# prequel-dev/plz4

Measured on AMD Instinct MI355X. Metric: MiB/s enc+dec, 4MiB independent blocks, level 1, block-checksum on (duplex steps over 2 streams), higher is better.
Workload: dtype u8

## Files before the change

plz4_amd/_native.py:

```python
from __future__ import annotations

import ctypes as C
import os

import numpy as np

HERE = os.path.dirname(os.path.abspath(__file__))
LIB_PATH = os.path.join(HERE, "libplz4hip.so")

ABI_VERSION = 2
SYMBOLS = [
    "plz4hip_abi_version", "plz4hip_device_count", "plz4hip_ctx_create", "plz4hip_ctx_destroy",
    "plz4hip_last_error", "plz4hip_compress_bound", "plz4hip_compress_batch", "plz4hip_decompress_batch",
    "plz4hip_xxh32_batch", "plz4hip_encode_records", "plz4hip_decode_records", "plz4hip_dev_stage_stride",
    "plz4hip_dev_encode_records", "plz4hip_dev_compact_records", "plz4hip_dev_scatter_records",
    "plz4hip_dev_decode_records", "plz4hip_dev_decode_records_ex", "plz4hip_dev_duplex_records", "plz4hip_dev_encode_body", "plz4hip_dev_duplex_body", "plz4hip_dev_encode_records_ex", "plz4hip_dev_encode_body_ex", "plz4hip_dev_compress", "plz4hip_dev_decompress", "plz4hip_ctx_trim",
    "plz4hip_ctx_counters",
    "plz4hip_dev_resident_waves", "plz4hip_dict_create", "plz4hip_dict_destroy", "plz4hip_compress_batch_dict", "plz4hip_decode_records_chains",
    "plz4hip_decompress_batch_dict", "plz4hip_encode_records_ex", "plz4hip_decode_records_ex",
    "plz4hip_xxh32_stream_create", "plz4hip_xxh32_stream_destroy", "plz4hip_xxh32_stream_reset", "plz4hip_xxh32_stream_update",
    "plz4hip_dev_xxh32_stream_update", "plz4hip_xxh32_stream_sum", "plz4hip_ctx_set_content_hash",
    "plz4hip_mgpu_create", "plz4hip_mgpu_destroy", "plz4hip_mgpu_count", "plz4hip_mgpu_ctx", "plz4hip_mgpu_last_error",
    "plz4hip_mgpu_compress_batch", "plz4hip_mgpu_decompress_batch", "plz4hip_mgpu_encode_records", "plz4hip_mgpu_decode_records",
    "plz4hip_mgpu_dev_encode_frame", "plz4hip_mgpu_dev_decode_frame",
# ... 363 lines not shown
    def hash_reset(self, h):
        self._chk(self.L.plz4hip_xxh32_stream_reset(self.h, h))

    def hash_update(self, h, buf: np.ndarray):
        buf = np.ascontiguousarray(buf)
        self._chk(self.L.plz4hip_xxh32_stream_update(self.h, h, buf.ctypes.data if buf.size else None, buf.size))

    def dev_hash_update(self, h, ptr, n, stream=0):
        self._chk(self.L.plz4hip_dev_xxh32_stream_update(self.h, h, ptr, n, stream))

    def hash_sum(self, h) -> int:
        out = C.c_uint32()
        self._chk(self.L.plz4hip_xxh32_stream_sum(self.h, h, C.byref(out)))
        return int(out.value)

    def set_content_hash(self, h):
        self._chk(self.L.plz4hip_ctx_set_content_hash(self.h, h))

    def trim(self):
        self._chk(self.L.plz4hip_ctx_trim(self.h))

    COUNTERS = ("fx_blocks", "fx_rounds_last", "fx_pieces_again", "dx_blocks", "dxl_blocks", "dxl_rounds_last", "dxl_groups_last",
                "fxl_blocks", "l1x_blocks", "hcx_blocks", "dx_big_blocks", "dx_big_rounds_last", "dx_big_runs_last",
                "mx_blocks", "mx_rounds_last", "mx_pieces_again", "mxl_blocks")

    def counters(self) -> dict:
        out = (C.c_int64 * len(self.COUNTERS))()
        rc = int(self.L.plz4hip_ctx_counters(self.h, out, len(self.COUNTERS)))
        if rc < 0:
            self._chk(rc)
        return {k: int(out[i]) for i, k in enumerate(self.COUNTERS)}


class MultiEngine:

    def __init__(self, devices):
        self.L = load()
        arr = (C.c_int * len(devices))(*devices)
        h = C.c_void_p()
        rc = self.L.plz4hip_mgpu_create(arr, len(devices), C.byref(h))
        if rc != 0:
            raise EngineError(rc, "plz4hip_mgpu_create")
        self.h = h
        self.g = len(devices)

    def close(self):
        if getattr(self, "h", None):
# ... 58 lines not shown
```

plz4_amd/csrc/plz4hip.hip:

```cpp
#include <hip/hip_runtime.h>

#include <array>
#include <atomic>
#include <mutex>
#include <thread>
#include <string>
#include <vector>
#include <cstdio>
#include <cstring>

#include "../../include/plz4hip.h"
#include "stream_ws.h"
#if defined(PLZ4_STATS)
__device__ unsigned long long plz4_stats[24];
#endif
#include "lz4_device.inl"
#include "lz4_seq_device.inl"
#include "lz4hc_device.inl"
#include "lz4hc12_device.inl"
#include "lz4hc_lazy_device.inl"
#include "lz4hcx_device.inl"
#include "lz4_dx_device.inl"
#include "lz4_fx_device.inl"
#include "lz4_mx_device.inl"
// ... 93 lines not shown
    ENC_WAVE_TABLE(lds);
    for (int i = next_block(a.queue); i < a.nBlocks; i = next_block(a.queue)) {
        const int      n   = block_len(a, i);
        const uint8_t* s   = a.src + (int64_t)i * a.srcStride;
        uint8_t*       rec = a.dst + (int64_t)i * a.dstStride;
        int      c    = wave_encode_block(s, n, rec + 4, a.bsz, lds);
        uint32_t word = (uint32_t)c & 0x7FFFFFFFu;
        if (c == 0) {
            wave_copy(rec + 4, s, n);
            c = n;
            word = 0x80000000u | ((uint32_t)n & 0x7FFFFFFFu);
        }
        int len = c + 4;
        if (a.blockChecksum) {
            WAVE_FENCE();
            const uint32_t x = wave_xxh32(rec + 4, c);
            if ((threadIdx.x & 63u) == 0) st32u(rec + 4 + c, x);
            len += 4;
        }
        if ((threadIdx.x & 63u) == 0) { st32u(rec, word); a.result[i] = len; }
    }
}

template <int kLdsWin = 0>
__device__ __forceinline__ void l1_parse_loop(const CodecArgs& a, uint32_t* lds, uint8_t* scr = nullptr)
{
    for (int i = next_block(a.queue); i < a.nBlocks; i = next_block(a.queue)) {
        const int gi = a.blk0 + i;
        const int n  = block_len(a, gi);
        int lastAnchor = 0, nseq = -1;
        if (n >= 0 && n <= a.l1MaxLen)
            nseq = wave_parse_l1<kLdsWin>(a.src + (int64_t)gi * a.srcStride, n, lds, a.l1Seq + (int64_t)i * a.l1SeqStride, &lastAnchor, scr);
        if ((threadIdx.x & 63u) == 0) { SeqInfo inf; inf.nseq = nseq; inf.lastAnchor = lastAnchor; inf.total = 0; inf.stored = 0; a.l1Info[i] = inf; }
    }
    if (a.gate && (threadIdx.x & 63u) == 0) atomicMax(a.gate, a.gateSeq);
}
__global__ __launch_bounds__(64) void k_parse_gate(const uint32_t* gate, uint32_t want)
{
    for (int it = 0; it < 400000; ++it) {
        if ((int32_t)(__hip_atomic_load(gate, __ATOMIC_RELAXED, __HIP_MEMORY_SCOPE_AGENT) - want) >= 0) break;
        __builtin_amdgcn_s_sleep(127);
    }
}
template <int W> __global__ __launch_bounds__(64 * W) void k_l1_parse(CodecArgs a)
{
    ENC_WAVE_TABLE(lds);
    l1_parse_loop<2>(a, lds);
}

template <bool kBack, bool kSeg = false> __device__ __forceinline__ void l1_sizes_body(const CodecArgs a, const FxlBlk* xb = nullptr)
{
    const int i = blockIdx.y, wave = blockIdx.x * 4 + (int)(threadIdx.x >> 6), nW = gridDim.x * 4;
    const int nseq = a.l1Info[i].nseq;
    if (nseq <= 0) return;
    const int gi = a.blk0 + i;
    const uint8_t*  s   = a.src + (int64_t)gi * a.srcStride;
    const uint64_t* seq = a.l1Seq + (int64_t)i * a.l1SeqStride;
    const int nChunks = (nseq + kSeqChunk - 1) / kSeqChunk;
    for (int c = wave; c < nChunks; c += nW) {
        const uint32_t v = seq_emit_sizes<kBack, kSeg>(s, seq, kBack ? a.l1Bk + (int64_t)i * a.l1SeqStride : nullptr, nseq, c, kSeg ? max_(xb[i].pfx, 0) : 0);
        if ((threadIdx.x & 63u) == 0) a.l1ChunkBytes[(int64_t)i * a.l1MaxChunks + c] = v;
    }
}
template <bool kBack> __global__ __launch_bounds__(256) void k_l1_sizes(CodecArgs a) { l1_sizes_body<kBack>(a); }

__global__ __launch_bounds__(256) void k_l1_scan(CodecArgs a)
{
    const int i = blockIdx.x * 4 + (int)(threadIdx.x >> 6);
    if (i >= a.nBlocks) return;
    const int gi = a.blk0 + i;
    const int n  = block_len(a, gi);
    SeqInfo inf = a.l1Info[i];
    const int cap = a.rawMode ? (a.dstCap ? a.dstCap[gi] : a.dstCapAll) : a.bsz;
    int total = 0;
    const bool broken = inf.nseq == kSeqEngineFailed;
    if (inf.nseq >= 0)
        total = seq_emit_scan(a.l1ChunkBytes + (int64_t)i * a.l1MaxChunks, a.l1ChunkOff + (int64_t)i * a.l1MaxChunks, inf.nseq, inf.lastAnchor, n, cap);
    if ((threadIdx.x & 63u) == 0) {
        inf.total = total; inf.stored = (total == 0);
        a.l1Info[i] = inf;
        if (broken) a.result[gi] = PLZ4HIP_E_DEVICE;
        else if (a.rawMode) a.result[gi] = total;
        else if (a.bodyOff) {
            a.result[gi] = (total ? total : n) + 4 + (a.blockChecksum ? 4 : 0);
        } else {
            const int c = total ? total : n;
            st32u(a.dst + (int64_t)gi * a.dstStride, total ? ((uint32_t)c & 0x7FFFFFFFu) : (0x80000000u | ((uint32_t)n & 0x7FFFFFFFu)));
// ... 1257 lines not shown
    wave_xxh32_x16(p, n, x);
    if ((threadIdx.x & 3u) == 0 && i < a.nBlocks) {
        const int st = n[0] < 0 ? PLZ4HIP_BLK_SIZE_OVERFLOW : x[0] != want ? PLZ4HIP_BLK_HASH_MISMATCH : PLZ4HIP_BLK_OK;
        a.status[i] = st;
        if (st != PLZ4HIP_BLK_OK) a.result[i] = 0;
    }
}
#if defined(PLZ4_EXP_DEC_EU)
__global__ __launch_bounds__(64) __attribute__((amdgpu_waves_per_eu(5, 6))) void k_decode_rec(CodecArgs a)
#else
__global__ __launch_bounds__(64) __attribute__((amdgpu_waves_per_eu(6, 6))) void k_decode_rec(CodecArgs a)
#endif
{
    __shared__ __attribute__((aligned(16))) uint8_t dl[kDecLdsBytes];
    decode_rec_loop<false>(a, dl);
}
__global__ __launch_bounds__(64) void k_decode_rec_dx(CodecArgs a)
{
    __shared__ __attribute__((aligned(16))) uint8_t dl[kDecLdsBytes];
    decode_rec_loop<true>(a, dl);
}

constexpr int kWinScratch = 256;
constexpr int duplex_wgs_per_cu(int P, int D) { return (160 * 1024) / (P * (kHashBytes + kWinScratch) + D * kDecLdsBytes); }
#if defined(PLZ4_EXP_DUPLEX_EU)
constexpr int duplex_waves_per_eu(int P, int D) { return PLZ4_EXP_DUPLEX_EU; }
#else
constexpr int duplex_waves_per_eu(int P, int D) { return ((P + D) * duplex_wgs_per_cu(P, D) + 3) / 4; }
#endif
template <int P, int D, int PRIO> __global__ __launch_bounds__(64 * (P + D))
__attribute__((amdgpu_waves_per_eu(duplex_waves_per_eu(P, D), duplex_waves_per_eu(P, D))))
void k_l1_duplex(CodecArgs a, CodecArgs d)
{
    __shared__ uint32_t tabS[P][kHashBytes / 4];
    __shared__ __attribute__((aligned(16))) uint8_t dlS[D][kDecLdsBytes];
    __shared__ __attribute__((aligned(16))) uint8_t winS[P][kWinScratch];
    const int w = plz4_readfirstlane((int)(threadIdx.x >> 6));
    if (w < P) {
        if (PRIO) __builtin_amdgcn_s_setprio(PRIO);
        l1_parse_loop<1>(a, tabS[w], winS[w]);
    } else {
        decode_rec_loop<false>(d, dlS[w - P]);
    }
}

__global__ __launch_bounds__(64) void k_xxh32(const uint8_t* base, int64_t stride, const int32_t* len, uint32_t* out,
                                              int n, uint32_t* queue)
{
    for (int i = next_block(queue); i < n; i = next_block(queue)) {
        const uint32_t x = wave_xxh32(base + (int64_t)i * stride, len[i]);
        if ((threadIdx.x & 63u) == 0) out[i] = x;
    }
}

__global__ __launch_bounds__(64) void k_xxh32_stream(XxhStream* st, const uint8_t* base, int64_t stride, const int32_t* lens, int n, int64_t single, int reset)
{
    if (reset) wave_xxh32_stream_reset(st);
    if (!lens) { wave_xxh32_stream_update(st, base, single); return; }
    for (int i = 0; i < n; ++i) {
        const int len = plz4_readfirstlane(lens[i]);
        if (len > 0) wave_xxh32_stream_update(st, base + (int64_t)i * stride, len);
    }
}

__global__ __launch_bounds__(64) void k_scan(const int32_t* __restrict__ len, int64_t* __restrict__ off, int n)
// ... 51 lines not shown
    int          cus = 0;
    int          encWaves = 0, decWaves = 0;
    struct HostSlot { uint8_t* h = nullptr; size_t hcap = 0; uint8_t* d = nullptr; size_t dcap = 0; hipStream_t s = nullptr;
                      hipEvent_t evData = nullptr, evHash = nullptr; bool hashBusy = false; DeviceBuffer l1; };
    plz4hip_xxh32_stream* contentHash = nullptr;
    static constexpr int kSlots = 3;
    HostSlot     slot[kSlots];
    DeviceBuffer hc;  int hcWaves = 0;
    DeviceBuffer h12;  int h12ParseWaves = 0;  int h12SegWaves = 0;  int hcLazyWaves = 0;  size_t h12ErrOff = 0;
    StreamOrder  hcOrder;
    hipStream_t  hashStream = nullptr;
    static constexpr int kL1Shared = 2;
    DeviceBuffer l1[kL1Shared];  StreamOrder l1Order[kL1Shared];
    int          l1Refused = 0;
    uint32_t*    d_gate = nullptr; uint32_t gateSeq = 0; hipStream_t gateStream = nullptr; bool gatePending = false; int gateBlocks = 0;
    hipStream_t  hcBuildStream = nullptr; hipEvent_t evHcFork = nullptr, evHcHist = nullptr, evHcChain[2] = {nullptr, nullptr}, evHcFree[2] = {nullptr, nullptr};
    DeviceBuffer hcPfx;  int hcLazyExWaves = 0;
    int hcxWaves[4] = {0, 0, 0, 0};
    DeviceBuffer dx;  StreamOrder dxOrder;
    hipStream_t  dxHashStream = nullptr; hipEvent_t evDxFork = nullptr, evDxHash = nullptr;
    DeviceBuffer fx;  StreamOrder fxOrder;
    DeviceBuffer mx;  StreamOrder mxOrder;
    DeviceBuffer xstage;  StreamOrder xstageOrder;
    static constexpr int kCounters = 17;
    unsigned long long* d_counters = nullptr;
    DeviceBuffer lenCopy;  StreamOrder lenOrder;
    DeviceBuffer chainCopy;  StreamOrder chainOrder;
    struct Owned { DeviceBuffer* buf; StreamOrder* order; bool trimmed; };
    std::array<Owned, 11> owned()
    {
        return {{{&hc, &hcOrder, true}, {&h12, &hcOrder, true}, {&hcPfx, &hcOrder, false}, {&l1[0], &l1Order[0], true},
                 {&l1[1], &l1Order[1], true}, {&dx, &dxOrder, true}, {&fx, &fxOrder, true}, {&lenCopy, &lenOrder, false},
                 {&chainCopy, &chainOrder, false}, {&xstage, &xstageOrder, true}, {&mx, &mxOrder, true}}};
    }
};

struct plz4hip_xxh32_stream { XxhStream* d_state = nullptr; hipEvent_t done = nullptr; };

struct plz4hip_dict {
    uint8_t*  d_bytes = nullptr;  int len = 0;
    uint32_t* d_table = nullptr;
    uint8_t*  d_hc = nullptr;
    uint8_t*  d_hcx = nullptr;
    std::vector<uint8_t> h_bytes;
};

namespace {

// ... 165 lines not shown
    a.l1Seq = (uint64_t*)a.h12F; a.l1SeqStride = L.fStride; a.l1MaxChunks = L.maxChunks; a.l1Bk = nullptr;
    a.l1Info = (SeqInfo*)(base + L.offInfo) + k;
    a.l1ChunkBytes = (uint32_t*)(base + L.offChunkB) + k * L.maxChunks; a.l1ChunkOff = (uint32_t*)(base + L.offChunkO) + k * L.maxChunks;
    a.lzRecStride = L.recStride;
    a.lzRec = (uint64_t*)(base + L.offRec) + k * L.recStride; a.lzBridge = (uint64_t*)(base + L.offBridge) + k * L.recStride;
    a.lzMeta = (LzSegMeta*)(base + L.offMeta) + k * kLzMaxSegs; a.lzStarts = (uint64_t*)(base + L.offStarts) + k * kLzMaxSegs * kLzStarts;
    a.lzPieces = (LzPiece*)(base + L.offPieces) + k * 2 * kLzMaxSegs;
}

void bind_hc_pre(CodecArgs& a, uint8_t* base, const HcPreLayout& L, bool lists)
{
    a.h12Chain = (uint16_t*)(base + L.offChain); a.h12ChainStride = L.stride;
    a.h12Rank = lists ? (uint32_t*)(base + L.offRank) : nullptr;
    a.h12List = lists ? (uint32_t*)(base + L.offList) : nullptr;
    a.h12Offsets = lists ? (uint32_t*)(base + L.offOffsets) : nullptr;
}

L1Switches read_l1_switches() { return parse_l1_switches([](const char* n) { return (const char*)getenv(n); }); }
MxSwitches read_mx_switches() { return parse_mx_switches([](const char* n) { return (const char*)getenv(n); }); }
HcSwitches read_hc_switches() { return parse_hc_switches([](const char* n) { return (const char*)getenv(n); }); }
DxSwitches read_dx_switches() { return parse_dx_switches([](const char* n) { return (const char*)getenv(n); }); }

enum class Emit { Back, Mid, Seg };
void launch_emit(hipStream_t s, const CodecArgs& a, int ng, int g0, int maxChunks, Emit kind, const FxlBlk* xb = nullptr, bool ctxSmall = false)
{
    int wg = (16384 / ng) / 4;
    if (wg > (maxChunks + 3) / 4) wg = (maxChunks + 3) / 4;
    if (wg < 1) wg = 1;
    if (kind == Emit::Seg) hipLaunchKernelGGL(k_fxl_sizes, dim3(wg, ng), dim3(256), 0, s, a, xb);
    else if (kind == Emit::Mid) hipLaunchKernelGGL(k_l1_sizes<false>, dim3(wg, ng), dim3(256), 0, s, a);
    else hipLaunchKernelGGL(k_l1_sizes<true>, dim3(wg, ng), dim3(256), 0, s, a);
    hipLaunchKernelGGL(k_l1_scan, dim3((ng + 3) / 4), dim3(256), 0, s, a);
    if (ctxSmall && a.bodyOff) hipLaunchKernelGGL(k_fxl_small, dim3(ng < 1024 ? ng : 1024), dim3(64), 0, s, a);
    if (a.bodyOff) hipLaunchKernelGGL(k_scan_from, dim3(1), dim3(64), 0, s, (const int32_t*)(a.result + g0), a.bodyOff + g0, ng, g0 == 0 ? 1 : 0);
    if (kind == Emit::Seg) hipLaunchKernelGGL(k_fxl_write, dim3(wg, ng), dim3(256), 0, s, a, xb);
    else if (kind == Emit::Mid) hipLaunchKernelGGL(k_l1_write<false>, dim3(wg, ng), dim3(256), 0, s, a);
    else hipLaunchKernelGGL(k_l1_write<true>, dim3(wg, ng), dim3(256), 0, s, a);
    if (!a.rawMode && a.blockChecksum) hipLaunchKernelGGL(k_l1_finish, dim3((ng + 15) / 16), dim3(64), 0, s, a);
    if (ctxSmall && !a.bodyOff) hipLaunchKernelGGL(k_fxl_small, dim3(ng < 1024 ? ng : 1024), dim3(64), 0, s, a);
}

void launch_rec_verify(hipStream_t s, const CodecArgs& d)
{
    if (d.blockChecksum && d.nBlocks > 0) hipLaunchKernelGGL(k_rec_verify16, dim3((d.nBlocks + 15) / 16), dim3(64), 0, s, d);
}
int launch_l1(plz4hip_ctx* c, hipStream_t s, CodecArgs a, int nb, int maxLen, int rawMode, DeviceBuffer* ws, bool* midDeclined = nullptr,
              const CodecArgs* rider = nullptr, bool hist = false, bool l1x = false, const L1Switches* read = nullptr);

int launch_hc_body(plz4hip_ctx* c, hipStream_t s, const HcSwitches& sw, CodecArgs a, int nb, int maxLen, int rawMode, bool* forked);
int launch_hc(plz4hip_ctx* c, hipStream_t s, CodecArgs a, int nb, int maxLen, int rawMode)
{
    const HcSwitches sw = read_hc_switches();
    HIPCHK(c, c->hcOrder.wait(s));
    MarkOnExit job;
// ... 249 lines not shown
{
    const int nws = sw.oneWorkspace ? 1 : plz4hip_ctx::kL1Shared;
    int mine = -1, idle = -1, fresh = -1;
    for (int i = 0; i < nws; ++i) {
        if (c->l1[i].d && c->l1Order[i].stream == s && mine < 0) mine = i;
        if (c->l1[i].d && idle < 0 && c->l1Order[i].idle()) idle = i;
        if (!c->l1[i].d && fresh < 0) fresh = i;
    }
    return mine >= 0 ? mine : (idle >= 0 ? idle : (fresh >= 0 ? fresh : 0));
}

int l1_gate(plz4hip_ctx* c, hipStream_t s, CodecArgs& a, int ng)
{
    if (c->gatePending && c->gateStream != s && c->gateBlocks >= 8 * c->cus)
        hipLaunchKernelGGL(k_parse_gate, dim3(1), dim3(64), 0, s, (const uint32_t*)c->d_gate, c->gateSeq);
    if (c->gateSeq >= 0x7FFF0000u) {
        HIPCHK(c, hipDeviceSynchronize()); HIPCHK(c, zero_sync(c, c->d_gate, sizeof(uint32_t))); c->gateSeq = 0;
    }
    a.gate = c->d_gate; a.gateSeq = ++c->gateSeq;
    c->gatePending = true; c->gateStream = s; c->gateBlocks = ng;
    return PLZ4HIP_OK;
}

int launch_duplex(plz4hip_ctx* c, hipStream_t s, const L1Switches& sw, const CodecArgs& a, const CodecArgs& rider, int ng)
{
    const int P = sw.duplexP, D = sw.duplexD;
#define DUPLEX_CASE(PP, DD) \
    if (P == PP && D == DD) { \
        int wgs = ((ng + PP - 1) / PP > (rider.nBlocks + DD - 1) / DD) ? (ng + PP - 1) / PP : (rider.nBlocks + DD - 1) / DD; \
        const int hold = c->cus * duplex_wgs_per_cu(PP, DD); \
        if (wgs > hold) wgs = hold; \
        if (sw.duplexPrio) hipLaunchKernelGGL((k_l1_duplex<PP, DD, 3>), dim3(wgs), dim3(64 * (PP + DD)), 0, s, a, rider); \
        else               hipLaunchKernelGGL((k_l1_duplex<PP, DD, 0>), dim3(wgs), dim3(64 * (PP + DD)), 0, s, a, rider); \
        return PLZ4HIP_OK; \
    }
    DUPLEX_CASE(1, 1) DUPLEX_CASE(1, 2) DUPLEX_CASE(3, 4) DUPLEX_CASE(9, 7)
#undef DUPLEX_CASE
    return fail(c, PLZ4HIP_E_ARG, "PLZ4HIP_DUPLEX: not a built combination");
}

int launch_l1(plz4hip_ctx* c, hipStream_t s, CodecArgs a, int nb, int maxLen, int rawMode, DeviceBuffer* ws, bool* midDeclined,
              const CodecArgs* rider, bool hist, bool l1x, const L1Switches* read)
{
    hipError_t e;
    const L1Switches sw = read ? *read : read_l1_switches();
    const bool mid = midDeclined != nullptr;
    const L1Shape shape{nb, maxLen, rawMode != 0, mid, rider != nullptr, hist, l1x, a.bodyOff != nullptr, hist && a.dictLen >= 8};
    const L1Want want = l1_want(shape, sw);
    const bool mxl = mid && a.hcPfx != nullptr;
    const MxShape mxShape{a.level, nb, maxLen, a.hcEx != 0 || a.hcPfx != nullptr, rider != nullptr};
    const MxWant mxWant = !mid ? MxWant{} : mxl ? mxl_want(mxShape, read_mx_switches()) : mx_want(mxShape, read_mx_switches());
    a.rawMode = rawMode; a.blk0 = 0; a.nBlocks = nb;
    const bool shared = (ws == nullptr);
    int wsi = 0;
    if (shared) { wsi = pick_l1_workspace(c, s, sw); ws = &c->l1[wsi]; }
    bool granted = want.staged;
    const auto need_for = [&](int per) { return l1_layout(per, maxLen, l1x).total; };
    int per = nb;
    if (shared && granted && wsi != 0 && !ws->d && c->l1Refused > 0) { c->l1Refused--; wsi = 0; ws = &c->l1[0]; }
    if (shared && granted && wsi != 0 && !ws->d) {
        bool refused = false;  HIPCHK(c, ws->reserve(need_for(nb), c->l1Order[wsi], &refused));
        if (refused) {
            wsi = 0; ws = &c->l1[0]; c->l1Refused = 8;
            if (getenv("PLZ4HIP_VERBOSE")) fprintf(stderr, "plz4hip: level 1: no room for a second workspace of %zu MiB, sharing the first\n", need_for(nb) >> 20);
        }
    }
    StreamOrder* const order = shared ? &c->l1Order[wsi] : nullptr;
    if (granted && need_for(nb) > ws->bytes) {
        size_t freeB = 0, totalB = 0;
        if (hipMemGetInfo(&freeB, &totalB) != hipSuccess) return fail(c, PLZ4HIP_E_DEVICE, "hipMemGetInfo");
        int rc = PLZ4HIP_OK;
        const int64_t grp = l1_first_group(freeB, ws->bytes, sw.budgetGiB, sw.budgetMiB, l1_layout(1, maxLen, l1x).perBlock, nb);
        const int got = fit_groups(nb, grp, false, [&](int p, bool* refused) {
            per = p;
            HIPCHK(c, order ? ws->reserve(need_for(per), *order, refused) : ws->reserve(need_for(per), s, refused));
            return (int)PLZ4HIP_OK;
        }, &rc);
        if (rc) return rc;
        if (!got) granted = false;
        if (getenv("PLZ4HIP_VERBOSE"))
            fprintf(stderr, "plz4hip: level 1, %d blocks of <= %d: free %zu MiB, workspace %zu MiB, groups of %d%s\n", nb, maxLen, freeB >> 20, ws->bytes >> 20, per, granted ? "" : " (fused)");
    }
    MarkOnExit job, pcJob;
    PieceArgs pc{};
    bool pcGranted = false;
    FxlBlk* xb = nullptr;
    L1Layout L{};
    if (granted) {
        if (order) { HIPCHK(c, order->wait(s)); job.arm(*order, s); }
        L = l1_layout(per, maxLen, l1x);
        a.l1MaxLen = maxLen;
        bind_l1(a, ws->d, L);
        const PieceCut cut = mid ? mxWant.cut() : want.cut();
        if (cut.on) {
            DeviceBuffer& buf = mid ? c->mx : c->fx;
            StreamOrder& ord = mid ? c->mxOrder : c->fxOrder;
            pc.pb = cut.piece; pc.warm = cut.warm; pc.P = cut.P; pc.recStride = piece_rec_stride(pc.pb); pc.cnt = c->d_counters;
            const bool blk = hist && !mid;
            const PieceLayout PL = piece_layout(per, pc.P, pc.recStride, mid ? kMxTab : kFxTab, blk);
            HIPCHK(c, ord.wait(s));
            bool refused = false;  HIPCHK(c, buf.reserve(PL.total, ord, &refused));
            if (!refused) { xb = bind_pieces(pc, buf.d, PL, blk); pcGranted = true; pcJob.arm(ord, s); }
        }
    }
    const L1Route route = l1_route(shape, sw, want, granted, pcGranted);
    const bool mxOn = route == L1Route::Mid && mx_route(mxWant, granted, pcGranted);
    switch (route) {
    case L1Route::NoMemBody:
        return fail(c, PLZ4HIP_E_NOMEM, "records straight into a frame body need the staged call's workspace (blocks up to 4 MiB)");
    case L1Route::MidDeclined:
        *midDeclined = true; return PLZ4HIP_OK;
    case L1Route::DictKernels: case L1Route::Fused:
        a.blk0 = 0; a.nBlocks = nb;
        a.queue = next_queue(c, s, &e); HIPCHK(c, e);
        if (route == L1Route::DictKernels) { if (rawMode) ENC_LAUNCH(k_encode_raw_dict, nb, c, s, a); else ENC_LAUNCH(k_encode_rec_dict, nb, c, s, a); }
        else                               { if (rawMode) ENC_LAUNCH(k_encode_raw, nb, c, s, a); else ENC_LAUNCH(k_encode_rec, nb, c, s, a); }
        if (route == L1Route::Fused && rider) { launch_rec_verify(s, *rider); hipLaunchKernelGGL(k_decode_rec, dim3(grid_for(rider->nBlocks, c->decWaves)), dim3(64), 0, s, *rider); }
        HIPCHK(c, hipGetLastError());
        HIPCHK(c, job.leave());
        HIPCHK(c, pcJob.leave());
        return PLZ4HIP_OK;
    default: break;
    }
    if (route == L1Route::L1x) xb = (FxlBlk*)(ws->d + L.offBlk);
    for (int g0 = 0; g0 < nb; g0 += per) {
        const int ng = nb - g0 < per ? nb - g0 : per;
        a.blk0 = g0; a.nBlocks = ng;
        a.queue = next_queue(c, s, &e); HIPCHK(c, e);
        if (rider && g0 == 0) launch_rec_verify(s, *rider);
        a.gate = nullptr;
        if (route == L1Route::Parse || route == L1Route::Duplex) {
            if (sw.noGate) c->gatePending = false;
            else if (int rc = l1_gate(c, s, a, ng)) return rc;
        } else if (route == L1Route::Mid) c->gatePending = false;
        switch (route) {
        case L1Route::Mid:
            if (mxOn && mxl) launch_piece_rounds<KMxl>(s, a, pc, xb, ng, g0 == 0);
            else if (mxOn) launch_piece_rounds<KMx>(s, a, pc, xb, ng, g0 == 0);
            else hipLaunchKernelGGL(hc_mid_kernel(a.hcPfx != nullptr), dim3(grid_for(ng, c->hcWaves)), dim3(64), 0, s, a);
            break;
        case L1Route::Fxl: launch_piece_rounds<KFxl>(s, a, pc, xb, ng, g0 == 0); break;
        case L1Route::Fx:  launch_piece_rounds<KFx>(s, a, pc, xb, ng, g0 == 0); break;
        case L1Route::L1x:
            ENC_LAUNCH(k_l1x_parse, ng, c, s, a, xb, c->d_counters);
            break;
        default:
            if (route == L1Route::Duplex && g0 == 0) { if (int rc = launch_duplex(c, s, sw, a, *rider, ng)) return rc; break; }
#if defined(PLZ4_EXP_TABBITS)
            {
            int W = 10; if (const char* ev = getenv("PLZ4HIP_EXP_W")) W = atoi(ev);
#define EXP_CASE(WW) if (W == WW) { int per = 0; hipOccupancyMaxActiveBlocksPerMultiprocessor(&per, k_l1_parse<WW>, 64 * WW, 0); \
                if (getenv("PLZ4HIP_VERBOSE")) fprintf(stderr, "exp: W=%d workgroups per CU %d\n", WW, per); \
                int wgs = c->cus * per; if (wgs * WW > ng) wgs = (ng + WW - 1) / WW; \
                hipLaunchKernelGGL(k_l1_parse<WW>, dim3(wgs), dim3(64 * WW), 0, s, a); }
            EXP_CASE(4) EXP_CASE(5) EXP_CASE(6) EXP_CASE(8) EXP_CASE(9) EXP_CASE(10) EXP_CASE(12) EXP_CASE(13) EXP_CASE(14) EXP_CASE(16)
#undef EXP_CASE
            }
#else
            ENC_LAUNCH(k_l1_parse, ng, c, s, a);
#endif
        }
        launch_emit(s, a, ng, g0, L.maxChunks, hist ? Emit::Seg : mid ? Emit::Mid : Emit::Back, xb, shape.ctx);
        HIPCHK(c, hipGetLastError());
    }
    HIPCHK(c, job.leave());
    HIPCHK(c, pcJob.leave());
    return PLZ4HIP_OK;
}

template <class Layout> void bind_dx_tables(CodecArgs& a, uint8_t* base, const Layout& L)
{
    a.dxT = (uint64_t*)(base + L.offT); a.dxTStride = (int64_t)L.tStride;
    a.dxPtr = (uint32_t*)(base + L.offPtr); a.dxPtrStride = (int64_t)L.pStride;
    a.dxUnits = (DxUnit*)(base + L.offUnits); a.dxMaxSeg = L.maxSeg;
    a.dxInfo = (DxInfo*)(base + L.offInfo);
}
void bind_dx(CodecArgs& a, uint8_t* base, const DxLayout& L, bool records, bool hashed, bool hist)
{
    bind_dx_tables(a, base, L);
    if (records) { a.dxSrcOff = (int64_t*)(base + L.offSrcOff); a.dxLen = (int32_t*)(base + L.offLen); }
    if (hashed) a.dxHashBad = (int32_t*)(base + L.offHashBad);
    if (!hist) return;
    a.dxlFirst = (int32_t*)(base + L.offFirst); a.dxlChain = (int32_t*)(base + L.offChain); a.dxlGood = (int32_t*)(base + L.offGood);
    a.dxlMoved = (uint32_t*)(base + L.offMoved);
}
// ... 155 lines not shown
void into_stage(CodecArgs& a, void* stage, int64_t stride) { a.dst = (uint8_t*)stage; a.dstStride = stride; a.bodyOff = nullptr; a.bodyCap = 0; }
void into_body(CodecArgs& a, void* body, int64_t bodyCap, int64_t* recOff) { a.dst = (uint8_t*)body; a.dstStride = 0; a.bodyOff = recOff; a.bodyCap = bodyCap; }
void dict_args(CodecArgs& a, const plz4hip_dict* dict) { a.dict = dict->d_bytes; a.dictLen = dict->len; a.dictTable = dict->d_table; }
void dict_hc_args(CodecArgs& a, const plz4hip_dict* dict, int level)
{
    const uint8_t* t = dict->d_hc + (level <= 2 ? 0 : (size_t)kHcWorkBytes);
    a.hcDictHash = (const uint32_t*)t; a.hcDictChain = (const uint16_t*)(t + kHcHashEntries * 4);
    a.hcxStart = (const uint32_t*)dict->d_hcx; a.hcxList = (const uint16_t*)(dict->d_hcx + kHcxDictStartBytes);
}

}

extern "C" {

int plz4hip_abi_version(void) { return PLZ4HIP_ABI_VERSION; }

#if defined(PLZ4_STATS)
int plz4hip_debug_stats(unsigned long long* out24)
{
    unsigned long long zero[24] = {0};
    if (hipDeviceSynchronize() != hipSuccess) return PLZ4HIP_E_DEVICE;
    if (hipMemcpyFromSymbol(out24, HIP_SYMBOL(plz4_stats), sizeof zero) != hipSuccess) return PLZ4HIP_E_DEVICE;
    if (hipMemcpyToSymbol(HIP_SYMBOL(plz4_stats), zero, sizeof zero) != hipSuccess) return PLZ4HIP_E_DEVICE;
    return PLZ4HIP_OK;
}
#endif

int plz4hip_device_count(void)
{
    int n = 0;
    if (hipGetDeviceCount(&n) != hipSuccess) return PLZ4HIP_E_DEVICE;
    return n;
}

int plz4hip_compress_bound(int n) { return ((unsigned)n > 0x7E000000u) ? 0 : n + n / 255 + 16; }

int64_t plz4hip_dev_stage_stride(int bsz) { return (int64_t)round_up((size_t)bsz + 8, 16); }

int plz4hip_ctx_create(int device, plz4hip_ctx** out)
{
    if (!out) return PLZ4HIP_E_ARG;
    *out = nullptr;
    int n = 0;
    if (hipGetDeviceCount(&n) != hipSuccess || device < 0 || device >= n) return PLZ4HIP_E_DEVICE;
    plz4hip_ctx* c = new (std::nothrow) plz4hip_ctx();
    if (!c) return PLZ4HIP_E_NOMEM;
// ... 856 lines not shown
```

plz4_amd/csrc/route.h:

```cpp
#pragma once
#include <climits>
#include <cstdio>
#include <cstdlib>
#include <vector>

namespace plz4 {

constexpr int kUnset = INT_MIN;

struct PieceCut { bool on; int piece, warm, P; };
inline PieceCut piece_cut(bool on, int maxLen, int pieceKiB, int warmKiB)
{
    PieceCut c{};
    c.on = on;
    if (on) { c.piece = pieceKiB << 10; c.warm = warmKiB << 10; c.P = (maxLen + c.piece - 1) / c.piece; }
    return c;
}
template <class Get> void parse_piece_kib(Get&& get, const char* pieceName, const char* warmName, int* pieceKiB, int* warmKiB)
{
    if (const char* v = get(pieceName)) { const int x = (int)atol(v); if (x >= 1 && x <= 4096) *pieceKiB = x; }
    if (const char* v = get(warmName)) { const int x = (int)atol(v); if (x >= 0 && x <= 4096) *warmKiB = x; }
}

constexpr int  kFxMaxBlocks = 128;
constexpr bool kL1xDefault = true;
struct L1Switches {
    bool fused = false;
    int  fxLinked = kUnset;
    int  fxMax = kFxMaxBlocks;
    int  fxPieceKiB = 64, fxWarmKiB = 64;
    int  l1x = kUnset;
    bool oneWorkspace = false;
    long budgetGiB = 0, budgetMiB = 0;
    bool noGate = false;
    int  duplexP = 1, duplexD = 1, duplexPrio = 3;
};

inline bool fxl_wanted(const L1Switches& sw, int nb, int maxLen)
{
    if (sw.fxLinked == 0) return false;
    return nb <= sw.fxMax && maxLen >= kFxMinLen && maxLen <= kSeqMaxBlock && !sw.fused;
}
inline bool l1x_on(const L1Switches& sw) { return !sw.fused && (sw.l1x == kUnset ? kL1xDefault : sw.l1x != 0); }

enum class L1Route { Fused, DictKernels, Parse, Duplex, Mid, Fx, Fxl, L1x, MidDeclined, NoMemBody };
struct L1Shape { int nb, maxLen; bool raw, mid, rider, hist, l1x, body, ctx; };
struct L1Want { bool staged, fx; int piece, warm, P; PieceCut cut() const { return PieceCut{fx, piece, warm, P}; } };
inline L1Want l1_want(const L1Shape& k, const L1Switches& sw)
{
    L1Want w{};
    const bool inRange = k.maxLen > 0 && k.maxLen <= kSeqMaxBlock && !sw.fused;
    const bool fxl = fxl_wanted(sw, k.nb, k.maxLen);
    w.staged = inRange && (!k.hist || fxl || (k.l1x && l1x_on(sw)));
    const bool fx = w.staged && !k.mid && !k.rider && k.nb <= sw.fxMax && k.maxLen >= kFxMinLen && k.maxLen <= kSeqMaxBlock && (!(k.hist || k.l1x) || fxl);
    const PieceCut c = piece_cut(fx, k.maxLen, sw.fxPieceKiB, sw.fxWarmKiB);
    w.fx = c.on; w.piece = c.piece; w.warm = c.warm; w.P = c.P;
    return w;
}
inline L1Route l1_route(const L1Shape& k, const L1Switches& sw, const L1Want& w, bool wsGranted, bool fxGranted)
// ... 169 lines not shown
    const bool dx = (w.dx || grouped) && granted;
    p.route = w.big && granted ? DxRoute::DxBig : !dx ? DxRoute::OneWave : grouped ? DxRoute::DxGrouped : DxRoute::Dx;
    p.tail = k.hist == kHistLinked ? (dx ? DxTail::None : DxTail::RecLinked)
           : k.hist ? (k.records ? DxTail::RecDict : DxTail::RawDict)
           : k.records ? (dx ? DxTail::RecDx : DxTail::Rec) : DxTail::Raw;
    return p;
}

template <class Get> L1Switches parse_l1_switches(Get&& get)
{
    const auto num = [&](const char* n, long unset) { const char* v = get(n); return v ? atol(v) : unset; };
    L1Switches sw;
    sw.fused = get("PLZ4HIP_L1_FUSED") != nullptr;
    sw.fxLinked = (int)num("PLZ4HIP_FX_LINKED", kUnset);
    if (const char* v = get("PLZ4HIP_FX_MAX_BLOCKS")) sw.fxMax = atoi(v);
    parse_piece_kib(get, "PLZ4HIP_FX_PIECE_KIB", "PLZ4HIP_FX_WARMUP_KIB", &sw.fxPieceKiB, &sw.fxWarmKiB);
    sw.l1x = (int)num("PLZ4HIP_L1X", kUnset);
    sw.oneWorkspace = num("PLZ4HIP_L1_WORKSPACES", 0) == 1;
    sw.budgetGiB = num("PLZ4HIP_L1_BUDGET_GIB", 0);
    sw.budgetMiB = num("PLZ4HIP_L1_BUDGET_MIB", 0);
    sw.noGate = get("PLZ4HIP_EXP_NO_GATE") != nullptr;
    if (const char* v = get("PLZ4HIP_DUPLEX")) { if (sscanf(v, "%d,%d", &sw.duplexP, &sw.duplexD) != 2) { sw.duplexP = 1; sw.duplexD = 1; } }
    sw.duplexPrio = (int)num("PLZ4HIP_DUPLEX_PRIO", 3);
    return sw;
}
template <class Get> HcSwitches parse_hc_switches(Get&& get)
{
    const auto num = [&](const char* n, long unset) { const char* v = get(n); return v ? atol(v) : unset; };
    const auto set = [&](const char* n) { return get(n) != nullptr; };
    HcSwitches sw;
    sw.hcx = (int)num("PLZ4HIP_HCX", kUnset);
    sw.extOff = set("PLZ4HIP_HC_EXT_OFF"); sw.midOff = set("PLZ4HIP_HC_MID_OFF"); sw.lazyOff = set("PLZ4HIP_HC_LAZY_OFF");
    sw.preOff = set("PLZ4HIP_HC_PRE_OFF"); sw.listsOff = set("PLZ4HIP_HC_LISTS_OFF");
    sw.h12Off = set("PLZ4HIP_HC12_OFF"); sw.h12Lazy = set("PLZ4HIP_HC12_LAZY"); sw.h12SegOff = set("PLZ4HIP_HC12_SEG_OFF");
    { const int m = (int)num("PLZ4HIP_HC_MIN_SEG", 0); if (m >= 64) sw.minSeg = m; }
    { const int n = (int)num("PLZ4HIP_HC_SEGS", kLzMaxSegs); sw.segs = n < 1 ? 1 : (n > kLzMaxSegs ? kLzMaxSegs : n); }
    sw.gather = (int)num("PLZ4HIP_HC12_GATHER", 12); sw.idle = (int)num("PLZ4HIP_HC12_IDLE", 16);
    sw.overlapMin = (int)num("PLZ4HIP_HC_OVERLAP_MIN", 2048);
    sw.overlapOff = set("PLZ4HIP_HC_OVERLAP_OFF");
    { const int w = (int)num("PLZ4HIP_HC_OVERLAP_GROUPS", 4); sw.overlapGroups = w < 2 ? 2 : w; }
    sw.budgetGiB = num("PLZ4HIP_HC_BUDGET_GIB", 0);
    sw.h12Group = (int)num("PLZ4HIP_HC12_GROUP", 0); sw.group = (int)num("PLZ4HIP_HC_GROUP", 0);
    return sw;
}
template <class Get> MxSwitches parse_mx_switches(Get&& get)
{
// ... 25 lines not shown
```

plz4_amd/csrc/ws_layout.h:

```cpp
#pragma once
#include <vector>

namespace plz4 {

inline size_t round_up(size_t v, size_t a) { return (v + a - 1) / a * a; }

struct WsTake { size_t off, count, size, align; };
struct Carver {
    std::vector<WsTake>* log = nullptr;
    size_t at = 0, perBlock = 0;
    template <class T> size_t take(size_t count, size_t align = 256)
    {
        const size_t off = at;
        at = off + round_up(count * sizeof(T), align);
        if (log) log->push_back({off, count, sizeof(T), alignof(T)});
        return off;
    }
    template <class T> size_t per_block(size_t blocks, size_t each, size_t align = 256)
    {
        perBlock += each * sizeof(T);
        return take<T>(blocks * each, align);
    }
};

// ... 20 lines not shown
    size_t budget = hc_default_budget(freeB + held);
    if (budgetGiB >= 1) budget = (size_t)budgetGiB << 30;
    return budget < held ? held : budget;
}

inline int64_t hc_first_group(size_t freeB, size_t held, long budgetGiB, int group, size_t perBlock, int nb)
{
    int64_t grp = (int64_t)(hc_budget(freeB, held, budgetGiB) / perBlock);
    if (group >= 1) grp = group;
    if (grp < 1) grp = 1;
    return grp > nb ? nb : grp;
}

inline int64_t l1_first_group(size_t freeB, size_t held, long budgetGiB, long budgetMiB, size_t perBlock, int nb)
{
    size_t budget = (freeB + held) / 2;
    if (budgetGiB >= 1) budget = (size_t)budgetGiB << 30;
    if (budgetMiB >= 1) budget = (size_t)budgetMiB << 20;
    if (budget < held) budget = held;
    const int64_t grp = (int64_t)(budget / (perBlock + 64));
    return grp > nb ? nb : grp;
}

struct L1Layout { size_t seqStride; int maxChunks; size_t perBlock, offInfo, offChunkBytes, offChunkOff, offSeq, offBk, offBlk, total; };
inline L1Layout l1_layout(int per, int maxLen, bool l1x, std::vector<WsTake>* log = nullptr)
{
    L1Layout L{};
    L.seqStride = round_up((size_t)(maxLen > 0 ? maxLen : 0) / 4 + 3, 64);
    L.maxChunks = (int)((L.seqStride + kSeqChunk - 1) / kSeqChunk);
    Carver c{log};
    const size_t n = (size_t)per;
    L.offInfo = c.per_block<SeqInfo>(n, 1);
    L.offChunkBytes = c.per_block<uint32_t>(n, (size_t)L.maxChunks);
    L.offChunkOff = c.per_block<uint32_t>(n, (size_t)L.maxChunks);
    L.offSeq = c.per_block<uint64_t>(n, L.seqStride, 8);
    L.offBk = c.per_block<uint8_t>(n, L.seqStride, 8);
    if (l1x) L.offBlk = c.per_block<FxlBlk>(n, 1, 1);
    L.perBlock = c.perBlock; L.total = c.at;
    return L;
}

struct PieceLayout { size_t offMeta, offIn, offOut, offRec, offBlk, total; };
inline PieceLayout piece_layout(int per, int P, int recStride, int tabWords, bool hist, std::vector<WsTake>* log = nullptr)
{
    PieceLayout L{};
    Carver c{log};
    const size_t nP = (size_t)per * (size_t)P;
    L.offMeta = c.take<PieceMeta>(nP);
    L.offIn = c.take<uint32_t>(nP * (size_t)tabWords, 4);
    L.offOut = c.take<uint32_t>(2 * nP * (size_t)tabWords, 4);
    L.offRec = c.take<uint64_t>(nP * (size_t)recStride, 8);
    L.offBlk = c.at;
    if (hist) L.offBlk = c.take<FxlBlk>((size_t)per);
    L.total = c.at;
    return L;
}
typedef PieceLayout FxLayout;
typedef PieceLayout MxLayout;
inline FxLayout fx_layout(int per, int P, int recStride, bool hist, std::vector<WsTake>* log = nullptr) { return piece_layout(per, P, recStride, kFxTab, hist, log); }
inline MxLayout mx_layout(int per, int P, int recStride, std::vector<WsTake>* log = nullptr) { return piece_layout(per, P, recStride, kMxTab, false, log); }
// ... 155 lines not shown
```

Baseline: 93240.

## Let idle duplex decode waves compute emit sizes for freshly parsed blocks

In the 1+1 duplex kernel, the parse wave posts each finished block index to an LDS mailbox ring. Once the decode wave finishes its own records, it takes those indices and runs the sequence-size emit for those blocks, then stamps a per-block mark. The later k_l1_sizes pass skips any block whose mark matches the current tag. The goal is to move sizing work into decode waves that would otherwise sit idle. The cost is extra LDS (kept to nine workgroups per CU), a marks buffer with a memset, fences and polling, and a new counter; a debug role-timestamp probe and a workgroup-cap knob are also added.

```diff
diff --git a/plz4_amd/_native.py b/plz4_amd/_native.py
--- a/plz4_amd/_native.py
+++ b/plz4_amd/_native.py
@@ -409,7 +409,7 @@
 
     COUNTERS = ("fx_blocks", "fx_rounds_last", "fx_pieces_again", "dx_blocks", "dxl_blocks", "dxl_rounds_last", "dxl_groups_last",
                 "fxl_blocks", "l1x_blocks", "hcx_blocks", "dx_big_blocks", "dx_big_rounds_last", "dx_big_runs_last",
-                "mx_blocks", "mx_rounds_last", "mx_pieces_again", "mxl_blocks")
+                "mx_blocks", "mx_rounds_last", "mx_pieces_again", "mxl_blocks", "duplex_sized_blocks")
 
     def counters(self) -> dict:
         out = (C.c_int64 * len(self.COUNTERS))()
diff --git a/plz4_amd/csrc/plz4hip.hip b/plz4_amd/csrc/plz4hip.hip
--- a/plz4_amd/csrc/plz4hip.hip
+++ b/plz4_amd/csrc/plz4hip.hip
@@ -139,8 +139,28 @@
     }
 }
 
-template <int kLdsWin = 0>
-__device__ __forceinline__ void l1_parse_loop(const CodecArgs& a, uint32_t* lds, uint8_t* scr = nullptr)
+constexpr int      kMbxRing = 8, kMbxPosted = kMbxRing, kMbxTaken = kMbxRing + 1, kMbxWords = kMbxRing + 4;
+constexpr uint32_t kMbxLeft = 0x80000000u;
+#define MBX_LOAD(p)     __hip_atomic_load((p), __ATOMIC_RELAXED, __HIP_MEMORY_SCOPE_WORKGROUP)
+#define MBX_STORE(p, v) __hip_atomic_store((p), (v), __ATOMIC_RELAXED, __HIP_MEMORY_SCOPE_WORKGROUP)
+__device__ __forceinline__ void mbx_post(uint32_t* mbx, int i)
+{
+    __builtin_amdgcn_fence(__ATOMIC_RELEASE, "agent");
+    if ((threadIdx.x & 63u) == 0) {
+        const uint32_t p = MBX_LOAD(&mbx[kMbxPosted]);
+        if (p - MBX_LOAD(&mbx[kMbxTaken]) < (uint32_t)kMbxRing) {
+            MBX_STORE(&mbx[p & (kMbxRing - 1)], (uint32_t)i);
+            __hip_atomic_store(&mbx[kMbxPosted], p + 1, __ATOMIC_RELEASE, __HIP_MEMORY_SCOPE_WORKGROUP);
+        }
+    }
+}
+__device__ __forceinline__ void mbx_leave(uint32_t* mbx)
+{
+    if ((threadIdx.x & 63u) == 0) MBX_STORE(&mbx[kMbxPosted], MBX_LOAD(&mbx[kMbxPosted]) | kMbxLeft);
+}
+
+template <int kLdsWin = 0, bool kPost = false>
+__device__ __forceinline__ void l1_parse_loop(const CodecArgs& a, uint32_t* lds, uint8_t* scr = nullptr, uint32_t* mbx = nullptr)
 {
     for (int i = next_block(a.queue); i < a.nBlocks; i = next_block(a.queue)) {
         const int gi = a.blk0 + i;
@@ -149,7 +169,9 @@
         if (n >= 0 && n <= a.l1MaxLen)
             nseq = wave_parse_l1<kLdsWin>(a.src + (int64_t)gi * a.srcStride, n, lds, a.l1Seq + (int64_t)i * a.l1SeqStride, &lastAnchor, scr);
         if ((threadIdx.x & 63u) == 0) { SeqInfo inf; inf.nseq = nseq; inf.lastAnchor = lastAnchor; inf.total = 0; inf.stored = 0; a.l1Info[i] = inf; }
-    }
+        if (kPost && mbx) mbx_post(mbx, i);
+    }
+    if (kPost && mbx) mbx_leave(mbx);
     if (a.gate && (threadIdx.x & 63u) == 0) atomicMax(a.gate, a.gateSeq);
 }
 __global__ __launch_bounds__(64) void k_parse_gate(const uint32_t* gate, uint32_t want)
@@ -165,9 +187,11 @@
     l1_parse_loop<2>(a, lds);
 }
 
-template <bool kBack, bool kSeg = false> __device__ __forceinline__ void l1_sizes_body(const CodecArgs a, const FxlBlk* xb = nullptr)
+template <bool kBack, bool kSeg = false> __device__ __forceinline__ void l1_sizes_body(const CodecArgs a, const FxlBlk* xb = nullptr,
+                                                                                       const uint32_t* marks = nullptr, uint32_t tag = 0)
 {
     const int i = blockIdx.y, wave = blockIdx.x * 4 + (int)(threadIdx.x >> 6), nW = gridDim.x * 4;
+    if (marks && marks[i] == tag) return;
     const int nseq = a.l1Info[i].nseq;
     if (nseq <= 0) return;
     const int gi = a.blk0 + i;
@@ -179,7 +203,10 @@
         if ((threadIdx.x & 63u) == 0) a.l1ChunkBytes[(int64_t)i * a.l1MaxChunks + c] = v;
     }
 }
-template <bool kBack> __global__ __launch_bounds__(256) void k_l1_sizes(CodecArgs a) { l1_sizes_body<kBack>(a); }
+template <bool kBack> __global__ __launch_bounds__(256) void k_l1_sizes(CodecArgs a, const uint32_t* marks, uint32_t tag)
+{
+    l1_sizes_body<kBack>(a, nullptr, kBack ? marks : nullptr, tag);
+}
 
 __global__ __launch_bounds__(256) void k_l1_scan(CodecArgs a)
 {
@@ -1483,25 +1510,84 @@
 }
 
 constexpr int kWinScratch = 256;
-constexpr int duplex_wgs_per_cu(int P, int D) { return (160 * 1024) / (P * (kHashBytes + kWinScratch) + D * kDecLdsBytes); }
+constexpr bool duplex_helps(int P, int D) { return P == 1 && D == 1; }
+constexpr int duplex_wgs_per_cu(int P, int D)
+{
+    return (160 * 1024) / (P * (kHashBytes + kWinScratch) + D * kDecLdsBytes + (duplex_helps(P, D) ? kMbxWords * 4 : 0));
+}
+static_assert(duplex_wgs_per_cu(1, 1) == 9, "the mailbox must leave nine 1 + 1 workgroups to a CU");
+
+struct DuplexHelp { uint32_t* marks; uint32_t tag; unsigned long long* cnt; };
+constexpr int kHelpPolls = 400000;
+__device__ __forceinline__ void duplex_help(const CodecArgs& a, const DuplexHelp& h, uint32_t* mbx)
+{
+    const bool lane0 = (threadIdx.x & 63u) == 0;
+    uint32_t taken = 0;
+    int sized = 0;
+    for (int polls = 0; polls < kHelpPolls; ) {
+        const uint32_t p = plz4_readfirstlane(lane0 ? MBX_LOAD(&mbx[kMbxPosted]) : 0u);
+        if (p & kMbxLeft) break;
+        if (p == taken) { __builtin_amdgcn_s_sleep(127); ++polls; continue; }
+        const int i = (int)plz4_readfirstlane(lane0 ? MBX_LOAD(&mbx[taken & (kMbxRing - 1)]) : 0u);
+        ++taken;
+        if (lane0) MBX_STORE(&mbx[kMbxTaken], taken);
+        __builtin_amdgcn_fence(__ATOMIC_ACQUIRE, "agent");
+        const int nseq = plz4_readfirstlane(__hip_atomic_load(&a.l1Info[i].nseq, __ATOMIC_RELAXED, __HIP_MEMORY_SCOPE_AGENT));
+        const int nChunks = nseq > 0 ? (nseq + kSeqChunk - 1) / kSeqChunk : 0;
+        const uint8_t*  s   = a.src + (int64_t)(a.blk0 + i) * a.srcStride;
+        const uint64_t* seq = a.l1Seq + (int64_t)i * a.l1SeqStride;
+        bool whole = true;
+        for (int c = 0; c < nChunks; ++c) {
+            if (plz4_readfirstlane(lane0 ? MBX_LOAD(&mbx[kMbxPosted]) : 0u) & kMbxLeft) { whole = false; break; }
+            const uint32_t v = seq_emit_sizes<true, false>(s, seq, a.l1Bk + (int64_t)i * a.l1SeqStride, nseq, c, 0);
+            if (lane0) a.l1ChunkBytes[(int64_t)i * a.l1MaxChunks + c] = v;
+        }
+        if (!whole) break;
+        __builtin_amdgcn_fence(__ATOMIC_RELEASE, "agent");
+        if (lane0) h.marks[i] = h.tag;
+        ++sized;
+    }
+    if (sized && lane0) atomicAdd(&h.cnt[17], (unsigned long long)sized);
+}
 #if defined(PLZ4_EXP_DUPLEX_EU)
 constexpr int duplex_waves_per_eu(int P, int D) { return PLZ4_EXP_DUPLEX_EU; }
 #else
 constexpr int duplex_waves_per_eu(int P, int D) { return ((P + D) * duplex_wgs_per_cu(P, D) + 3) / 4; }
 #endif
+#if defined(PLZ4_ROLE_TS)
+constexpr unsigned long long kRoleTsInv = 1ull << 62;
+__device__ unsigned long long plz4_role_ts[512 * 12];
+#define ROLE_TS(a, b, start) do { if ((a).gate && (threadIdx.x & 63u) == 0) { \
+        unsigned long long* r_ = plz4_role_ts + ((a).gateSeq & 511u) * 12; const unsigned long long t_ = wall_clock64(); \
+        atomicMax(&r_[b], kRoleTsInv - t_); \
+        if (!(start)) { atomicMax(&r_[(b) + 1], t_); atomicAdd(&r_[(b) + 2], t_); atomicAdd(&r_[(b) + 3], 1ull); } } } while (0)
+#else
+#define ROLE_TS(a, b, start) do {} while (0)
+#endif
 template <int P, int D, int PRIO> __global__ __launch_bounds__(64 * (P + D))
 __attribute__((amdgpu_waves_per_eu(duplex_waves_per_eu(P, D), duplex_waves_per_eu(P, D))))
-void k_l1_duplex(CodecArgs a, CodecArgs d)
+void k_l1_duplex(CodecArgs a, CodecArgs d, DuplexHelp h)
 {
     __shared__ uint32_t tabS[P][kHashBytes / 4];
     __shared__ __attribute__((aligned(16))) uint8_t dlS[D][kDecLdsBytes];
     __shared__ __attribute__((aligned(16))) uint8_t winS[P][kWinScratch];
+    constexpr bool kHelp = duplex_helps(P, D);
+    __shared__ uint32_t mbxS[kHelp ? kMbxWords : 1];
     const int w = plz4_readfirstlane((int)(threadIdx.x >> 6));
+    ROLE_TS(a, 0, true);
+    if (kHelp) {
+        if (threadIdx.x < (unsigned)kMbxWords) mbxS[threadIdx.x] = 0;
+        __syncthreads();
+    }
+    uint32_t* const mbx = kHelp && h.marks ? mbxS : nullptr;
     if (w < P) {
         if (PRIO) __builtin_amdgcn_s_setprio(PRIO);
-        l1_parse_loop<1>(a, tabS[w], winS[w]);
+        l1_parse_loop<1, kHelp>(a, tabS[w], winS[w], mbx);
+        ROLE_TS(a, 5, false);
     } else {
         decode_rec_loop<false>(d, dlS[w - P]);
+        ROLE_TS(a, 1, false);
+        if (kHelp && mbx) duplex_help(a, h, mbx);
     }
 }
 
@@ -1599,8 +1685,9 @@
     DeviceBuffer fx;  StreamOrder fxOrder;
     DeviceBuffer mx;  StreamOrder mxOrder;
     DeviceBuffer xstage;  StreamOrder xstageOrder;
-    static constexpr int kCounters = 17;
+    static constexpr int kCounters = 18;
     unsigned long long* d_counters = nullptr;
+    uint32_t helpTag = 0;
     DeviceBuffer lenCopy;  StreamOrder lenOrder;
     DeviceBuffer chainCopy;  StreamOrder chainOrder;
     struct Owned { DeviceBuffer* buf; StreamOrder* order; bool trimmed; };
@@ -1812,14 +1899,15 @@
 DxSwitches read_dx_switches() { return parse_dx_switches([](const char* n) { return (const char*)getenv(n); }); }
 
 enum class Emit { Back, Mid, Seg };
-void launch_emit(hipStream_t s, const CodecArgs& a, int ng, int g0, int maxChunks, Emit kind, const FxlBlk* xb = nullptr, bool ctxSmall = false)
+void launch_emit(hipStream_t s, const CodecArgs& a, int ng, int g0, int maxChunks, Emit kind, const FxlBlk* xb = nullptr, bool ctxSmall = false,
+                 const uint32_t* marks = nullptr, uint32_t tag = 0)
 {
     int wg = (16384 / ng) / 4;
     if (wg > (maxChunks + 3) / 4) wg = (maxChunks + 3) / 4;
     if (wg < 1) wg = 1;
     if (kind == Emit::Seg) hipLaunchKernelGGL(k_fxl_sizes, dim3(wg, ng), dim3(256), 0, s, a, xb);
-    else if (kind == Emit::Mid) hipLaunchKernelGGL(k_l1_sizes<false>, dim3(wg, ng), dim3(256), 0, s, a);
-    else hipLaunchKernelGGL(k_l1_sizes<true>, dim3(wg, ng), dim3(256), 0, s, a);
+    else if (kind == Emit::Mid) hipLaunchKernelGGL(k_l1_sizes<false>, dim3(wg, ng), dim3(256), 0, s, a, (const uint32_t*)nullptr, 0u);
+    else hipLaunchKernelGGL(k_l1_sizes<true>, dim3(wg, ng), dim3(256), 0, s, a, marks, tag);
     hipLaunchKernelGGL(k_l1_scan, dim3((ng + 3) / 4), dim3(256), 0, s, a);
     if (ctxSmall && a.bodyOff) hipLaunchKernelGGL(k_fxl_small, dim3(ng < 1024 ? ng : 1024), dim3(64), 0, s, a);
     if (a.bodyOff) hipLaunchKernelGGL(k_scan_from, dim3(1), dim3(64), 0, s, (const int32_t*)(a.result + g0), a.bodyOff + g0, ng, g0 == 0 ? 1 : 0);
@@ -2115,7 +2203,7 @@
     return PLZ4HIP_OK;
 }
 
-int launch_duplex(plz4hip_ctx* c, hipStream_t s, const L1Switches& sw, const CodecArgs& a, const CodecArgs& rider, int ng)
+int launch_duplex(plz4hip_ctx* c, hipStream_t s, const L1Switches& sw, const CodecArgs& a, const CodecArgs& rider, int ng, const DuplexHelp& h)
 {
     const int P = sw.duplexP, D = sw.duplexD;
 #define DUPLEX_CASE(PP, DD) \
@@ -2123,8 +2211,9 @@
         int wgs = ((ng + PP - 1) / PP > (rider.nBlocks + DD - 1) / DD) ? (ng + PP - 1) / PP : (rider.nBlocks + DD - 1) / DD; \
         const int hold = c->cus * duplex_wgs_per_cu(PP, DD); \
         if (wgs > hold) wgs = hold; \
-        if (sw.duplexPrio) hipLaunchKernelGGL((k_l1_duplex<PP, DD, 3>), dim3(wgs), dim3(64 * (PP + DD)), 0, s, a, rider); \
-        else               hipLaunchKernelGGL((k_l1_duplex<PP, DD, 0>), dim3(wgs), dim3(64 * (PP + DD)), 0, s, a, rider); \
+        if (sw.duplexWgs >= 1 && wgs > sw.duplexWgs) wgs = sw.duplexWgs; \
+        if (sw.duplexPrio) hipLaunchKernelGGL((k_l1_duplex<PP, DD, 3>), dim3(wgs), dim3(64 * (PP + DD)), 0, s, a, rider, h); \
+        else               hipLaunchKernelGGL((k_l1_duplex<PP, DD, 0>), dim3(wgs), dim3(64 * (PP + DD)), 0, s, a, rider, h); \
         return PLZ4HIP_OK; \
     }
     DUPLEX_CASE(1, 1) DUPLEX_CASE(1, 2) DUPLEX_CASE(3, 4) DUPLEX_CASE(9, 7)
@@ -2148,7 +2237,8 @@
     int wsi = 0;
     if (shared) { wsi = pick_l1_workspace(c, s, sw); ws = &c->l1[wsi]; }
     bool granted = want.staged;
-    const auto need_for = [&](int per) { return l1_layout(per, maxLen, l1x).total; };
+    const bool marks = rider != nullptr && !mid && !hist && duplex_help_on(sw);
+    const auto need_for = [&](int per) { return l1_layout(per, maxLen, l1x, nullptr, marks).total; };
     int per = nb;
     if (shared && granted && wsi != 0 && !ws->d && c->l1Refused > 0) { c->l1Refused--; wsi = 0; ws = &c->l1[0]; }
     if (shared && granted && wsi != 0 && !ws->d) {
@@ -2163,7 +2253,7 @@
         size_t freeB = 0, totalB = 0;
         if (hipMemGetInfo(&freeB, &totalB) != hipSuccess) return fail(c, PLZ4HIP_E_DEVICE, "hipMemGetInfo");
         int rc = PLZ4HIP_OK;
-        const int64_t grp = l1_first_group(freeB, ws->bytes, sw.budgetGiB, sw.budgetMiB, l1_layout(1, maxLen, l1x).perBlock, nb);
+        const int64_t grp = l1_first_group(freeB, ws->bytes, sw.budgetGiB, sw.budgetMiB, l1_layout(1, maxLen, l1x, nullptr, marks).perBlock, nb);
         const int got = fit_groups(nb, grp, false, [&](int p, bool* refused) {
             per = p;
             HIPCHK(c, order ? ws->reserve(need_for(per), *order, refused) : ws->reserve(need_for(per), s, refused));
@@ -2181,7 +2271,7 @@
     L1Layout L{};
     if (granted) {
         if (order) { HIPCHK(c, order->wait(s)); job.arm(*order, s); }
-        L = l1_layout(per, maxLen, l1x);
+        L = l1_layout(per, maxLen, l1x, nullptr, marks);
         a.l1MaxLen = maxLen;
         bind_l1(a, ws->d, L);
         const PieceCut cut = mid ? mxWant.cut() : want.cut();
@@ -2220,6 +2310,13 @@
         const int ng = nb - g0 < per ? nb - g0 : per;
         a.blk0 = g0; a.nBlocks = ng;
         a.queue = next_queue(c, s, &e); HIPCHK(c, e);
+        DuplexHelp help{nullptr, 0u, c->d_counters};
+        if (marks && route == L1Route::Duplex && g0 == 0) {
+            help.marks = (uint32_t*)(ws->d + L.offMark);
+            if (++c->helpTag == 0) c->helpTag = 1;
+            help.tag = c->helpTag;
+            HIPCHK(c, hipMemsetAsync(help.marks, 0, round_up((size_t)ng * 4, 16), s));
+        }
         if (rider && g0 == 0) launch_rec_verify(s, *rider);
         a.gate = nullptr;
         if (route == L1Route::Parse || route == L1Route::Duplex) {
@@ -2238,7 +2335,7 @@
             ENC_LAUNCH(k_l1x_parse, ng, c, s, a, xb, c->d_counters);
             break;
         default:
-            if (route == L1Route::Duplex && g0 == 0) { if (int rc = launch_duplex(c, s, sw, a, *rider, ng)) return rc; break; }
+            if (route == L1Route::Duplex && g0 == 0) { if (int rc = launch_duplex(c, s, sw, a, *rider, ng, help)) return rc; break; }
 #if defined(PLZ4_EXP_TABBITS)
             {
             int W = 10; if (const char* ev = getenv("PLZ4HIP_EXP_W")) W = atoi(ev);
@@ -2253,7 +2350,7 @@
             ENC_LAUNCH(k_l1_parse, ng, c, s, a);
 #endif
         }
-        launch_emit(s, a, ng, g0, L.maxChunks, hist ? Emit::Seg : mid ? Emit::Mid : Emit::Back, xb, shape.ctx);
+        launch_emit(s, a, ng, g0, L.maxChunks, hist ? Emit::Seg : mid ? Emit::Mid : Emit::Back, xb, shape.ctx, help.marks, help.tag);
         HIPCHK(c, hipGetLastError());
     }
     HIPCHK(c, job.leave());
@@ -2455,6 +2552,17 @@
     if (hipDeviceSynchronize() != hipSuccess) return PLZ4HIP_E_DEVICE;
     if (hipMemcpyFromSymbol(out24, HIP_SYMBOL(plz4_stats), sizeof zero) != hipSuccess) return PLZ4HIP_E_DEVICE;
     if (hipMemcpyToSymbol(HIP_SYMBOL(plz4_stats), zero, sizeof zero) != hipSuccess) return PLZ4HIP_E_DEVICE;
+    return PLZ4HIP_OK;
+}
+#endif
+
+#if defined(PLZ4_ROLE_TS)
+int plz4hip_debug_role_ts(unsigned long long* out)
+{
+    static unsigned long long zero[512 * 12];
+    if (hipDeviceSynchronize() != hipSuccess) return PLZ4HIP_E_DEVICE;
+    if (hipMemcpyFromSymbol(out, HIP_SYMBOL(plz4_role_ts), sizeof zero) != hipSuccess) return PLZ4HIP_E_DEVICE;
+    if (hipMemcpyToSymbol(HIP_SYMBOL(plz4_role_ts), zero, sizeof zero) != hipSuccess) return PLZ4HIP_E_DEVICE;
     return PLZ4HIP_OK;
 }
 #endif
diff --git a/plz4_amd/csrc/route.h b/plz4_amd/csrc/route.h
--- a/plz4_amd/csrc/route.h
+++ b/plz4_amd/csrc/route.h
@@ -24,6 +24,7 @@
 
 constexpr int  kFxMaxBlocks = 128;
 constexpr bool kL1xDefault = true;
+constexpr bool kDuplexHelpDefault = true;
 struct L1Switches {
     bool fused = false;
     int  fxLinked = kUnset;
@@ -34,7 +35,10 @@
     long budgetGiB = 0, budgetMiB = 0;
     bool noGate = false;
     int  duplexP = 1, duplexD = 1, duplexPrio = 3;
-};
+    bool duplexHelp = kDuplexHelpDefault;
+    int  duplexWgs = 0;
+};
+inline bool duplex_help_on(const L1Switches& sw) { return sw.duplexHelp && sw.duplexP == 1 && sw.duplexD == 1; }
 
 inline bool fxl_wanted(const L1Switches& sw, int nb, int maxLen)
 {
@@ -250,6 +254,8 @@
     sw.noGate = get("PLZ4HIP_EXP_NO_GATE") != nullptr;
     if (const char* v = get("PLZ4HIP_DUPLEX")) { if (sscanf(v, "%d,%d", &sw.duplexP, &sw.duplexD) != 2) { sw.duplexP = 1; sw.duplexD = 1; } }
     sw.duplexPrio = (int)num("PLZ4HIP_DUPLEX_PRIO", 3);
+    if (const char* v = get("PLZ4HIP_DUPLEX_HELP")) sw.duplexHelp = atol(v) != 0;
+    sw.duplexWgs = (int)num("PLZ4HIP_DUPLEX_WGS", 0);
     return sw;
 }
 template <class Get> HcSwitches parse_hc_switches(Get&& get)
diff --git a/plz4_amd/csrc/ws_layout.h b/plz4_amd/csrc/ws_layout.h
--- a/plz4_amd/csrc/ws_layout.h
+++ b/plz4_amd/csrc/ws_layout.h
@@ -66,8 +66,8 @@
     return grp > nb ? nb : grp;
 }
 
-struct L1Layout { size_t seqStride; int maxChunks; size_t perBlock, offInfo, offChunkBytes, offChunkOff, offSeq, offBk, offBlk, total; };
-inline L1Layout l1_layout(int per, int maxLen, bool l1x, std::vector<WsTake>* log = nullptr)
+struct L1Layout { size_t seqStride; int maxChunks; size_t perBlock, offInfo, offChunkBytes, offChunkOff, offSeq, offBk, offBlk, total, offMark; };
+inline L1Layout l1_layout(int per, int maxLen, bool l1x, std::vector<WsTake>* log = nullptr, bool marks = false)
 {
     L1Layout L{};
     L.seqStride = round_up((size_t)(maxLen > 0 ? maxLen : 0) / 4 + 3, 64);
@@ -80,6 +80,7 @@
     L.offSeq = c.per_block<uint64_t>(n, L.seqStride, 8);
     L.offBk = c.per_block<uint8_t>(n, L.seqStride, 8);
     if (l1x) L.offBlk = c.per_block<FxlBlk>(n, 1, 1);
+    if (marks) { c.at = round_up(c.at, 16); L.offMark = c.per_block<uint32_t>(n, 1, 16); }
     L.perBlock = c.perBlock; L.total = c.at;
     return L;
 }
```

Result: no change. 93480 (median of 6 runs) (+0.3%).
